# wavey-ai/soundkit

Hardware: AMD Instinct MI355X
Metric: AAC-LC 1024-sample frames/s (whole node) + xrealtime, batch=4096 48 kHz stereo (higher is better)
Workload: dtype f32 (synthesis f32; s16 between the kernels as in the reference; FIR: the 16-bit samples as 2 x f16 exactly, the f32 taps as 2 x f16 to 2^-24, f32 accumulate; 1.0e-7 rel. RMS vs f64)

## Files before the change

soundkit_amd/csrc/fir_bf16.hip:

```cpp
#include "sk_device.h"

#include <cstdlib>
#include <type_traits>

namespace sk {

namespace {

typedef float f32x4 __attribute__((ext_vector_type(4)));
typedef __bf16 bf16x8 __attribute__((ext_vector_type(8)));
typedef uint32_t u32x4 __attribute__((ext_vector_type(4)));
typedef uint32_t u32x2 __attribute__((ext_vector_type(2)));

constexpr int kRing = 192;
constexpr int kPlaneBytes = 2 * kRing;
__host__ __device__ constexpr int row_bytes(int planes) { return planes * kPlaneBytes + 32; }
constexpr int kWindows = 10;
__device__ constexpr int kProducts[kWindows] = {1, 3, 6, 6, 6, 6, 6, 3, 3, 1};
__host__ __device__ constexpr int products_of(int s, bool in16) { return in16 && kProducts[s] > 5 ? 5 : kProducts[s]; }
__device__ constexpr int kProductsF16[kWindows] = {kFirProductsF16[0], kFirProductsF16[1], kFirProductsF16[2], kFirProductsF16[3], kFirProductsF16[4],
                                                     kFirProductsF16[5], kFirProductsF16[6], kFirProductsF16[7], kFirProductsF16[8], kFirProductsF16[9]};
__host__ __device__ constexpr int products_of(int s, bool in16, bool f16) { return f16 ? kProductsF16[s] : products_of(s, in16); }
#ifndef SK_BF_AHEAD
#define SK_BF_AHEAD 3
#endif
constexpr int kAhead = SK_BF_AHEAD;

__host__ __device__ constexpr int ring_index(int rho) { return ((rho % kRing) + kRing) % kRing; }

template <bool PACKED>
__device__ __forceinline__ size_t row_base_offset(const FirArgs &a, uint32_t row) {
    if (!PACKED) return (size_t)row * a.in_stride;
    const uint32_t sh = a.in_ch - 1;
    return (size_t)(row >> sh) * a.in_group_stride + (size_t)((row & sh) << 10);
}

template <bool PACKED>
__device__ __forceinline__ size_t time_offset(const FirArgs &a, uint32_t i) {
    return PACKED ? (size_t)(i >> 10) * a.in_block_stride + (size_t)(i & 1023) : (size_t)i;
}

__device__ __forceinline__ void split_pair(float x0, float x1, uint32_t &p1, uint32_t &p2, uint32_t &p3) {
    const uint32_t u0 = __float_as_uint(x0), u1 = __float_as_uint(x1);
    p1 = __builtin_amdgcn_perm(u1, u0, 0x07060302u);
    const float r0 = x0 - __uint_as_float(u0 & 0xffff0000u), r1 = x1 - __uint_as_float(u1 & 0xffff0000u);
    const uint32_t v0 = __float_as_uint(r0), v1 = __float_as_uint(r1);
    p2 = __builtin_amdgcn_perm(v1, v0, 0x07060302u);
    const float s0 = r0 - __uint_as_float(v0 & 0xffff0000u), s1 = r1 - __uint_as_float(v1 & 0xffff0000u);
    p3 = __builtin_amdgcn_perm(__float_as_uint(s1), __float_as_uint(s0), 0x07060302u);
}

__device__ __forceinline__ void split_pair16(uint32_t u, uint32_t &p1, uint32_t &p2) {
    const uint32_t m = u & 0xff00ff00u;
    const float a0 = (float)(int)(int16_t)(m & 0xffffu), a1 = (float)((int)m >> 16);
    const float b0 = (float)(u & 0xffu), b1 = (float)((u >> 16) & 0xffu);
    p1 = __builtin_amdgcn_perm(__float_as_uint(a1), __float_as_uint(a0), 0x07060302u);
    p2 = __builtin_amdgcn_perm(__float_as_uint(b1), __float_as_uint(b0), 0x07060302u);
}

__device__ __forceinline__ void split_pair16_f16(uint32_t u, uint32_t &p1, uint32_t &p2) { dev_split_pair16_f16(u, p1, p2); }

template <bool IN16>
struct Stage {
    using Elem = std::conditional_t<IN16, int16_t, float>;
    using Vec = std::conditional_t<IN16, u32x2, f32x4>;
    const Elem *base[4];
    uint32_t ok_mask;
    Vec v[2 * kAhead];
};

template <bool ALIGNED, bool PACKED, bool IN16>
__device__ __forceinline__ void stage_init(const FirArgs &a, int lane, uint32_t row0, Stage<IN16> &st) {
    st.ok_mask = 0;
    if (ALIGNED) {
#pragma unroll
        for (int ld = 0; ld < 4; ++ld) {
            const uint32_t r = row0 + 4 * ld + (lane >> 4);
            const bool ok = r < a.rows;
            const uint32_t phys = a.row_map ? a.row_map[ok ? r : 0] : (ok ? r : 0);
            if constexpr (IN16) st.base[ld] = a.in16 + row_base_offset<PACKED>(a, phys) + 4 * (lane & 15);
            else st.base[ld] = a.in + row_base_offset<PACKED>(a, phys) + 4 * (lane & 15);
            if (ok) st.ok_mask |= 1u << ld;
        }
    }
}

template <bool ALIGNED, bool PACKED, bool INTERIOR = false, bool IN16 = false>
__device__ __forceinline__ void stage_issue(const FirArgs &a, int lane, uint32_t row0, int64_t n, Stage<IN16> &st, int half, int slot) {
    using Vec = typename Stage<IN16>::Vec;
    using Elem = typename Stage<IN16>::Elem;
    if (ALIGNED) {
        const int64_t c0 = n - a.in_origin;
        const bool inside = c0 >= 0 && c0 + 64 <= (int64_t)a.in_frames;
        const bool one_block = !PACKED || (((uint32_t)c0 & 1023u) + 64u <= 1024u);
        if (INTERIOR || __builtin_expect(inside && one_block, 1)) {
            const size_t off = time_offset<PACKED>(a, (uint32_t)c0);
#pragma unroll
            for (int e2 = 0; e2 < 2; ++e2) {
                const int ld = 2 * half + e2, sl = 2 * slot + e2;
                st.v[sl] = *reinterpret_cast<const Vec *>(st.base[ld] + off);
            }
        } else {
            asm volatile("; chunk at an edge of the row" ::: "memory");
            const int64_t idx = c0 + 4 * (lane & 15);
            const bool in_range = (uint64_t)idx + 3 < (uint64_t)a.in_frames;
            const ptrdiff_t off = (ptrdiff_t)time_offset<PACKED>(a, (uint32_t)idx) - 4 * (lane & 15);
            const uint32_t sel = in_range ? st.ok_mask : 0u;
#pragma unroll
            for (int e2 = 0; e2 < 2; ++e2) {
                const int ld = 2 * half + e2, sl = 2 * slot + e2;
                const Elem *src = ((sel >> ld) & 1u) ? st.base[ld] + off : reinterpret_cast<const Elem *>(a.zeros) + 4 * lane;
                st.v[sl] = *reinterpret_cast<const Vec *>(src);
            }
        }
    } else if constexpr (!IN16) {
        const int64_t idx = n + lane - a.in_origin;
        const bool in_range = idx >= 0 && idx < (int64_t)a.in_frames;
        const size_t off = time_offset<PACKED>(a, (uint32_t)idx);
#pragma unroll
        for (int e2 = 0; e2 < 2; ++e2) {
            const int ld = 2 * half + e2, sl = 2 * slot + e2;
#pragma unroll
            for (int e = 0; e < 4; ++e) {
                const uint32_t r = row0 + 4 * ld + e;
                const bool ok = in_range && r < a.rows;
                const uint32_t phys = a.row_map ? a.row_map[r < a.rows ? r : 0] : r;
                st.v[sl][e] = ok ? a.in[row_base_offset<PACKED>(a, phys) + off] : 0.0f;
            }
        }
    }
}

template <bool ALIGNED, bool IN16, bool F16 = false>
__device__ __forceinline__ void stage_commit(unsigned char *lds, int lane, int ring_at, const Stage<IN16> &st, int half, int slot) {
#pragma unroll
    for (int e2 = 0; e2 < 2; ++e2) {
        const int ld = 2 * half + e2, sl = 2 * slot + e2;
        if constexpr (IN16) {
            uint32_t p1a, p2a, p1b, p2b;
            if constexpr (F16) {
                split_pair16_f16(st.v[sl][0], p1a, p2a);
                split_pair16_f16(st.v[sl][1], p1b, p2b);
            } else {
                split_pair16(st.v[sl][0], p1a, p2a);
                split_pair16(st.v[sl][1], p1b, p2b);
            }
            unsigned char *dst = lds + (4 * ld + (lane >> 4)) * row_bytes(2) + 2 * (ring_at + 4 * (lane & 15));
            *reinterpret_cast<u32x2 *>(dst) = (u32x2){p1a, p1b};
            *reinterpret_cast<u32x2 *>(dst + kPlaneBytes) = (u32x2){p2a, p2b};
        } else if (ALIGNED) {
            uint32_t p1a, p2a, p3a, p1b, p2b, p3b;
            split_pair(st.v[sl][0], st.v[sl][1], p1a, p2a, p3a);
            split_pair(st.v[sl][2], st.v[sl][3], p1b, p2b, p3b);
            unsigned char *dst = lds + (4 * ld + (lane >> 4)) * row_bytes(3) + 2 * (ring_at + 4 * (lane & 15));
            *reinterpret_cast<u32x2 *>(dst) = (u32x2){p1a, p1b};
            *reinterpret_cast<u32x2 *>(dst + kPlaneBytes) = (u32x2){p2a, p2b};
            *reinterpret_cast<u32x2 *>(dst + 2 * kPlaneBytes) = (u32x2){p3a, p3b};
        } else {
#pragma unroll
            for (int e = 0; e < 4; ++e) {
                uint32_t p1, p2, p3;
                split_pair(st.v[sl][e], 0.0f, p1, p2, p3);
                unsigned char *dst = lds + (4 * ld + e) * row_bytes(3) + 2 * (ring_at + lane);
                *reinterpret_cast<uint16_t *>(dst) = (uint16_t)p1;
                *reinterpret_cast<uint16_t *>(dst + kPlaneBytes) = (uint16_t)p2;
                *reinterpret_cast<uint16_t *>(dst + 2 * kPlaneBytes) = (uint16_t)p3;
            }
        }
    }
}

struct BFrag {
    u32x4 p[3];
};

__device__ __forceinline__ f32x4 mfma_bf16(const u32x4 &av, const u32x4 &bv, const f32x4 &c) {
    return dev_mfma_bf16(av, bv, c);
}

__device__ __forceinline__ f32x4 mfma_f16(const u32x4 &av, const u32x4 &bv, const f32x4 &c) { return dev_mfma_f16(av, bv, c); }

template <bool ALIGNED, bool PACKED, int OUT16, bool IN16 = false, bool F16 = false>
#ifndef SK_FIR_F16_WAVES
#define SK_FIR_F16_WAVES 3
#endif
__global__ __launch_bounds__(64, F16 ? SK_FIR_F16_WAVES : 2) void k_fir_48k_16k_bf16(FirArgs a, int32_t pair0, int32_t pair_end, int32_t pairs_per_seg,
                                                            uint32_t n_segs, int out_vec) {
    static_assert(!IN16 || ALIGNED, "s16 rows are read four samples at a time");
    static_assert(!F16 || IN16, "the f16 planes exist for s16 rows");
    constexpr int kPlanes = IN16 ? 2 : 3;
    __shared__ __attribute__((aligned(16))) unsigned char lds[16 * row_bytes(kPlanes)];

    const int lane = threadIdx.x;
    const int j = lane & 15, q = lane >> 4;
    const uint32_t group = blockIdx.x / n_segs, seg = blockIdx.x % n_segs;
    const uint32_t row0 = group * 16;
    const int32_t p_begin = pair0 + (int32_t)seg * pairs_per_seg;
    const int32_t p_end = p_begin + pairs_per_seg < pair_end ? p_begin + pairs_per_seg : pair_end;
    if (p_begin >= p_end) return;
    const int32_t p_last = p_end + 3;

    u32x4 af[kWindows][3];
    {
        const u32x4 *src = reinterpret_cast<const u32x4 *>(F16 ? a.afrag_f16 : a.afrag16);
        constexpr int kTapPlanes = F16 ? 2 : 3;
#pragma unroll
        for (int s = 0; s < kWindows; ++s)
#pragma unroll
            for (int k = 0; k < kTapPlanes; ++k) af[s][k] = src[(s * kTapPlanes + k) * 64 + lane];
    }

    Stage<IN16> st;
    stage_init<ALIGNED, PACKED, IN16>(a, lane, row0, st);

    const int64_t n_begin = (int64_t)96 * p_begin;
#pragma unroll
    for (int c = -2; c < 0; ++c) {
        stage_issue<ALIGNED, PACKED, false, IN16>(a, lane, row0, n_begin + 64 * c, st, 0, 0);
        stage_issue<ALIGNED, PACKED, false, IN16>(a, lane, row0, n_begin + 64 * c, st, 1, 1);
        stage_commit<ALIGNED, IN16, F16>(lds, lane, ring_index(64 * c), st, 0, 0);
        stage_commit<ALIGNED, IN16, F16>(lds, lane, ring_index(64 * c), st, 1, 1);
    }
#pragma unroll
    for (int i = 0; i < kAhead; ++i) stage_issue<ALIGNED, PACKED, false, IN16>(a, lane, row0, n_begin + 64 * (i >> 1), st, i & 1, i % kAhead);

    const uint32_t out_row = row0 + j;
    float *out_ptr = OUT16 ? nullptr
                           : a.out + (size_t)(out_row < a.rows ? out_row : 0) * a.out_stride +
                                 ((a.out_off && out_row < a.rows) ? a.out_off[out_row] : 0);

    const unsigned char *b_base = lds + j * row_bytes(kPlanes) + 16 * q;
    const unsigned char *b_base_wrap = b_base - (q >= 2 ? 2 * kRing : 0);
    auto read_b = [&](int rho) __attribute__((always_inline)) {
        BFrag f;
        const unsigned char *src = (ring_index(rho) + 32 > kRing ? b_base_wrap : b_base) + 2 * ring_index(rho);
#pragma unroll
        for (int p = 0; p < kPlanes; ++p) f.p[p] = *reinterpret_cast<const u32x4 *>(src + p * kPlaneBytes);
        return f;
    };

    const bool row_exists = out_row < a.rows;
    constexpr bool to_s16 = OUT16 != 0;
    float *out_lane = to_s16 ? nullptr : out_ptr + 4 * q;
    int16_t *out16_ptr = to_s16 ? a.out16 + (size_t)((row_exists ? out_row : 0) / (OUT16 ? OUT16 : 1)) * a.out16_stride * OUT16 : nullptr;
    auto store_tile = [&](auto itag, const f32x4 &vraw, int32_t pair, int parity) __attribute__((always_inline)) {
        const f32x4 v = F16 ? vraw * (1.0f / 2147483648.0f) : (IN16 ? vraw * (1.0f / 32768.0f) : vraw);
        constexpr bool INTERIOR = decltype(itag)::value;
        if (!INTERIOR && (pair < p_begin || pair >= p_end)) return;
        const int32_t rel_tile = 32 * pair + 16 * parity - (int32_t)a.out_first;
        const bool whole = INTERIOR || (out_vec && rel_tile >= 0 && rel_tile + 16 <= (int32_t)a.out_count);
        const bool row_ok = INTERIOR || row_exists;
        const int32_t rel = rel_tile + 4 * q;
        if (!to_s16) {
            if (INTERIOR || __builtin_expect(whole, 1)) {
                if (row_ok) *reinterpret_cast<f32x4 *>(out_lane + rel_tile) = v;
            } else {
                asm volatile("; tile at an edge of the output, or unaligned rows" ::: "memory");
#pragma unroll
                for (int r = 0; r < 4; ++r)
                    if (row_ok && rel + r >= 0 && rel + r < (int32_t)a.out_count) out_ptr[rel + r] = v[r];
            }
            return;
        }
        uint32_t mine01, mine23;
        if constexpr (IN16) {
            mine01 = dev_pack2_s16_scaled<F16 ? 31 : 15>(vraw[0], vraw[1]);
            mine23 = dev_pack2_s16_scaled<F16 ? 31 : 15>(vraw[2], vraw[3]);
        } else {
            mine01 = dev_pack2_s16(v[0], v[1]);
            mine23 = dev_pack2_s16(v[2], v[3]);
        }
        if (OUT16 == 2) {
            const uint32_t other01 = (uint32_t)__builtin_amdgcn_update_dpp(0, (int)mine01, 0xB1, 0xF, 0xF, true);
            const uint32_t other23 = (uint32_t)__builtin_amdgcn_update_dpp(0, (int)mine23, 0xB1, 0xF, 0xF, true);
            uint32_t w[4];
            w[0] = (mine01 & 0xffffu) | (other01 << 16);
            w[1] = (mine01 >> 16) | (other01 & 0xffff0000u);
            w[2] = (mine23 & 0xffffu) | (other23 << 16);
            w[3] = (mine23 >> 16) | (other23 & 0xffff0000u);
            if ((j & 1) == 0 && row_ok) {
                uint32_t *dst = reinterpret_cast<uint32_t *>(out16_ptr) + rel;
                if (INTERIOR || __builtin_expect(whole, 1)) {
                    *reinterpret_cast<u32x4 *>(dst) = (u32x4){w[0], w[1], w[2], w[3]};
                } else {
                    asm volatile("; tile at an edge of the output, or unaligned rows" ::: "memory");
#pragma unroll
                    for (int r = 0; r < 4; ++r)
                        if (rel + r >= 0 && rel + r < (int32_t)a.out_count) dst[r] = w[r];
                }
            }
        } else if (row_ok) {
            int16_t *dst = out16_ptr + rel;
            if (INTERIOR || __builtin_expect(whole, 1)) {
                *reinterpret_cast<u32x2 *>(dst) = (u32x2){mine01, mine23};
            } else {
                asm volatile("; tile at an edge of the output, or unaligned rows" ::: "memory");
#pragma unroll
                for (int r = 0; r < 4; ++r)
                    if (rel + r >= 0 && rel + r < (int32_t)a.out_count) dst[r] = (int16_t)((r < 2 ? mine01 : mine23) >> (16 * (r & 1)));
            }
        }
    };

    f32x4 acc[2][4];
#pragma unroll
    for (int par = 0; par < 2; ++par)
#pragma unroll
        for (int b = 0; b < 4; ++b) acc[par][b] = (f32x4){0.f, 0.f, 0.f, 0.f};

    BFrag bcur = read_b(-128);

    auto period = [&](auto ktag, auto itag, int32_t P, int64_t n_body) __attribute__((always_inline)) {
        constexpr int K = decltype(ktag)::value;
        constexpr bool INTERIOR = decltype(itag)::value;
#pragma unroll
        for (int wi = 0; wi < 3; ++wi) {
            const int step = 3 * K + wi;
            {
                __builtin_amdgcn_sched_barrier(0);
                stage_commit<ALIGNED, IN16, F16>(lds, lane, ring_index(64 * (step >> 1)), st, step & 1, step % kAhead);
                stage_issue<ALIGNED, PACKED, INTERIOR, IN16>(a, lane, row0, n_body + 64 * ((step + kAhead) >> 1), st,
                                                             (step + kAhead) & 1, step % kAhead);
            }
#pragma unroll
            for (int par = 0; par < 2; ++par) {
                const int t = 32 * step;
                const int rho_next = par == 0 ? t - 80 : t + 32 - 128;
                const BFrag bnext = read_b(rho_next);
#pragma unroll
                for (int prod = 0; prod < 6; ++prod) {
                    constexpr int hk[6] = {0, 1, 0, 1, 2, 0};
                    constexpr int xk[6] = {0, 0, 1, 1, 0, 2};
#pragma unroll
                    for (int d = 0; d < 4; ++d) {
                        const int s = 3 * d + wi;
                        if (s >= kWindows || prod >= products_of(s, IN16, F16)) continue;
                        f32x4 &c = acc[par][(K - d + 4) & 3];
                        const f32x4 c0 = (s == 0 && prod == 0) ? (f32x4){0.f, 0.f, 0.f, 0.f} : c;
                        if constexpr (F16) c = mfma_f16(af[s][hk[prod]], bcur.p[xk[prod]], c0);
                        else c = mfma_bf16(af[s][hk[prod]], bcur.p[xk[prod]], c0);
                    }
                }
                if (wi == 1 && par == 0) {
                    store_tile(itag, acc[0][(K + 1) & 3], P - 3, 0);
                    store_tile(itag, acc[1][(K + 1) & 3], P - 3, 1);
                }
                bcur = bnext;
            }
            if (INTERIOR) {
                int mfmas = 0;
#pragma unroll
                for (int d = 0; d < 4; ++d)
                    if (3 * d + wi < kWindows) mfmas += 2 * products_of(3 * d + wi, IN16, F16);
#pragma unroll
                for (int g = 0; g < mfmas; ++g) {
                    __builtin_amdgcn_sched_group_barrier(0x008, 1, 0);
                    __builtin_amdgcn_sched_group_barrier(0x002, 2, 0);
                }
            }
        }
    };

    using K0 = std::integral_constant<int, 0>;
    using K1 = std::integral_constant<int, 1>;
    using K2 = std::integral_constant<int, 2>;
    using K3 = std::integral_constant<int, 3>;
    const bool chunks_in_blocks = !PACKED || ((uint32_t)(n_begin - a.in_origin) & 63u) == 0;
    auto is_interior = [&](int32_t P0) {
        const int64_t n_body = (int64_t)96 * P0;
        const int64_t c_first = n_body + 64 * (kAhead >> 1) - a.in_origin, c_end = n_body + 64 * ((11 + kAhead) >> 1) + 64 - a.in_origin;
        const int64_t rel_first = (int64_t)32 * (P0 - 3) - (int64_t)a.out_first, rel_end = (int64_t)32 * P0 + 32 - (int64_t)a.out_first;
        return ALIGNED && chunks_in_blocks && c_first >= 0 && c_end <= (int64_t)a.in_frames && P0 - 3 >= p_begin && P0 < p_end &&
               out_vec && rel_first >= 0 && rel_end <= (int64_t)a.out_count && row0 + 16 <= a.rows;
    };
    auto general_body = [&](int32_t P0) __attribute__((always_inline)) {
        const int64_t n_body = (int64_t)96 * P0;
        if (P0 + 0 < p_last) period(K0{}, std::false_type{}, P0 + 0, n_body);
        if (P0 + 1 < p_last) period(K1{}, std::false_type{}, P0 + 1, n_body);
        if (P0 + 2 < p_last) period(K2{}, std::false_type{}, P0 + 2, n_body);
        if (P0 + 3 < p_last) period(K3{}, std::false_type{}, P0 + 3, n_body);
    };
    int32_t P0 = p_begin;
    for (; P0 < p_last && !is_interior(P0); P0 += 4) general_body(P0);
    for (; P0 < p_last && is_interior(P0); P0 += 4) {
        const int64_t n_body = (int64_t)96 * P0;
        period(K0{}, std::true_type{}, P0 + 0, n_body);
        period(K1{}, std::true_type{}, P0 + 1, n_body);
        period(K2{}, std::true_type{}, P0 + 2, n_body);
        period(K3{}, std::true_type{}, P0 + 3, n_body);
    }
    for (; P0 < p_last; P0 += 4) general_body(P0);
}

}

static bool fir_bf16_supported(const FirArgs &a) {
    const int64_t end_pair = ((int64_t)a.out_first + a.out_count + 31) / 32;
    return a.afrag16 != nullptr && end_pair <= 0x7ffffff0ll / 96 && a.out_count <= 0x7fffff00u;
}

hipError_t launch_fir_48k_16k(const FirArgs &a, hipStream_t s) {
    if (a.rows == 0 || a.out_count == 0) return hipSuccess;
    if (!fir_bf16_supported(a)) return hipErrorInvalidValue;
    const uint32_t groups = (a.rows + 15) / 16;
    const int64_t first_pair = ((int64_t)a.out_first / 32) & ~(int64_t)3;
    const int64_t end_pair = ((int64_t)a.out_first + a.out_count + 31) / 32;
    if (end_pair > 0x7ffffff0ll / 96 || a.out_count > 0x7fffff00u) return hipErrorInvalidValue;
    const uint32_t pairs = (uint32_t)(end_pair - first_pair);
    static const bool f16_rows = [] { const char *v = std::getenv("SK_FIR_S16_BF16"); return !(v && v[0] == '1'); }();
    const uint32_t waves_target = (a.in16 && a.afrag_f16 && f16_rows) ? 1024u * SK_FIR_F16_WAVES : 2048u;
    uint32_t n_segs = (waves_target + groups - 1) / groups;
    const uint32_t max_segs = pairs / 16 ? pairs / 16 : 1;
    if (n_segs > max_segs) n_segs = max_segs;
    uint32_t pps = (pairs + n_segs - 1) / n_segs;
    pps = (pps + 3) & ~3u;
    n_segs = (pairs + pps - 1) / pps;

    const bool strides_ok = a.in_block ? (a.in_block % 4 == 0 && a.in_block_stride % 4 == 0 && a.in_group_stride % 4 == 0)
                                       : (a.in_stride % 4 == 0);
    const bool aligned = ((a.in_origin & 3) == 0) && strides_ok && (a.in_frames % 4 == 0) &&
                         (a.in16 ? (((uintptr_t)a.in16 & 7) == 0) : (((uintptr_t)a.in & 15) == 0));
    if (a.out16 && (a.out16_ch < 1 || a.out16_ch > 2 || a.out_off || a.rows % a.out16_ch)) return hipErrorInvalidValue;
    const int out_vec = a.out16 ? ((a.out_first % 4 == 0) && (a.out16_stride * a.out16_ch) % 8 == 0 && (((uintptr_t)a.out16 & 15) == 0))
                                : ((a.out_first % 4 == 0) && (a.out_stride % 4 == 0) && (((uintptr_t)a.out & 15) == 0) &&
                                   a.out_off == nullptr);
    const bool packed = a.in_block != 0;
    if (packed && (a.in_block != 1024 || a.in_ch < 1 || a.in_ch > 2)) return hipErrorInvalidValue;
    const dim3 grid(groups * n_segs), block(64);
#define SK_FIR_LAUNCH(AL, PK, O16)                                                                                 \
    hipLaunchKernelGGL((k_fir_48k_16k_bf16<AL, PK, O16>), grid, block, 0, s, a, (int32_t)first_pair, (int32_t)end_pair, \
                       (int32_t)pps, n_segs, out_vec)
    if (a.in16) {
        if (!packed || !aligned) return hipErrorInvalidValue;
        const bool use_f16 = f16_rows;
#define SK_FIR_LAUNCH16(O16, F)                                                                                                    \
    hipLaunchKernelGGL((k_fir_48k_16k_bf16<true, true, O16, true, F>), grid, block, 0, s, a, (int32_t)first_pair, (int32_t)end_pair, \
                       (int32_t)pps, n_segs, out_vec)
        if (use_f16 && a.afrag_f16) {
            if (!a.out16) SK_FIR_LAUNCH16(0, true);
            else if (a.out16_ch == 2) SK_FIR_LAUNCH16(2, true);
            else SK_FIR_LAUNCH16(1, true);
        } else {
            if (!a.out16) SK_FIR_LAUNCH16(0, false);
            else if (a.out16_ch == 2) SK_FIR_LAUNCH16(2, false);
            else SK_FIR_LAUNCH16(1, false);
        }
#undef SK_FIR_LAUNCH16
    } else if (a.out16) {
        if (!packed) return hipErrorInvalidValue;
        if (aligned && a.out16_ch == 2) SK_FIR_LAUNCH(true, true, 2);
        else if (aligned) SK_FIR_LAUNCH(true, true, 1);
        else if (a.out16_ch == 2) SK_FIR_LAUNCH(false, true, 2);
        else SK_FIR_LAUNCH(false, true, 1);
    } else if (aligned && packed) SK_FIR_LAUNCH(true, true, 0);
    else if (aligned) SK_FIR_LAUNCH(true, false, 0);
    else if (packed) SK_FIR_LAUNCH(false, true, 0);
    else SK_FIR_LAUNCH(false, false, 0);
#undef SK_FIR_LAUNCH
    return hipGetLastError();
}

}
```

soundkit_amd/csrc/sk_device.h:

```cpp
#pragma once
#include <hip/hip_runtime.h>
#include <stdint.h>

#include "../../include/soundkit_amd.h"
#include "mp3_codebook_blob.h"

namespace sk {

struct SynthEntry {
    uint32_t off1024;
    uint32_t win;
};

struct SynthTask {
    uint32_t state;
    uint32_t begin;
    uint32_t count;
    uint32_t pad;
};

struct SynthTables {
    const float2 *tw_long;
    const float2 *tw_short;
    const float2 *w64;
    const float2 *w512;
    const float *win;
};

struct SynthArgs {
    const float *coeffs;
    float *pcm;
    int16_t *pcm16;
    float *delay;
    uint8_t *prev_shape;
    const SynthTask *tasks;
    const SynthEntry *entries;
    uint32_t n_tasks;
    uint32_t only_long;
    SynthTables t;
};

struct FrameSpan {
    uint32_t off1024;
    uint32_t channels;
};

hipError_t launch_aac_synth(const SynthArgs &a, hipStream_t s);
struct TailArgs {
    SynthArgs s;
    const uint32_t *afrag_f16;
    int16_t *out16;
    size_t out_stride;
    size_t stream_stride;
};
hipError_t launch_aac_tail(const TailArgs &ta, hipStream_t s);
hipError_t launch_aac_synth_pairs(const SynthArgs &a, bool with_short, hipStream_t s);
hipError_t launch_reset_streams(float *delay, uint8_t *shape, uint32_t *pns, const uint32_t *ids, uint32_t n, hipStream_t s);
hipError_t launch_zero_spans(float *base, const uint32_t *ids, uint32_t n, uint32_t span_floats, hipStream_t s);
hipError_t launch_frames_to_s16(const float *planar, int16_t *out, const FrameSpan *frames, uint32_t n, hipStream_t s);
hipError_t launch_dequantize(const int16_t *q, const int16_t *sf, float *out, size_t n, const float *pow43,
                             const float *sftab, hipStream_t s);

hipError_t launch_pcm_convert(int op, const void *in, void *out, size_t n, hipStream_t s);
hipError_t launch_interleave(const void *planar, void *out, size_t frames, uint32_t ch, int elem_bytes, hipStream_t s);
hipError_t launch_deinterleave(const void *in, void *planar, size_t frames, uint32_t ch, int elem_bytes, hipStream_t s);
hipError_t launch_deinterleave_s24(const uint8_t *in, int32_t *planar, size_t frames, uint32_t ch, hipStream_t s);
hipError_t launch_bytes_to_f32_planar(int variant, int fmt, const uint8_t *in, size_t frames, uint32_t ch, float *planar,
                                      hipStream_t s);
hipError_t launch_f32_planar_to_bytes(int fmt, const float *planar, size_t frames, uint32_t ch, uint8_t *out,
                                      hipStream_t s);
hipError_t launch_downmix_mono(const float *planar, size_t frames, uint32_t ch, float *mono, hipStream_t s);
hipError_t launch_exact_to_i16(int fmt, const uint8_t *in, size_t samples, uint8_t *out, hipStream_t s);
hipError_t launch_f32_planar_to_bytes_batch(int fmt, const float *planar, size_t batch, size_t plane_stride, size_t frames,
                                            uint32_t ch, uint8_t *out, hipStream_t s);

#ifdef __HIPCC__
__device__ __forceinline__ int dev_float_sample_to_i16(float x) {
    const float f = isfinite(x) ? fminf(fmaxf(x, -1.0f), 1.0f) : 0.0f;
    const double scaled = f < 0.0f ? (double)f * 32768.0 : (double)f * 32767.0;
    const int r = (int)round(scaled);
    return r < -32768 ? -32768 : (r > 32767 ? 32767 : r);
}

__device__ __forceinline__ int dev_float_sample_to_i16_f32(float x) {
    const float m = isfinite(x) ? fminf(fabsf(x), 1.0f) : 0.0f;
    const float a = m * 32768.0f;
    const float k = floorf(a);
    const float d = a - k;
    const int ki = (int)k;
    const int neg = ki + (d >= 0.5f ? 1 : 0);
    const int pos = ki + ((d - 0.5f >= m) ? 1 : 0) - ((d + 0.5f < m) ? 1 : 0);
    return x < 0.0f ? -neg : pos;
}
__device__ __forceinline__ int dev_float_sample_to_i16_v2(float x) {
    const float m = isfinite(x) ? fminf(fabsf(x), 1.0f) : 0.0f;
    const float a = m * 32768.0f;
    const float d = __builtin_amdgcn_fractf(a);
    const int ki = (int)a;
    const float mm = x < 0.0f ? 0.0f : m;
    const int r = ki + ((d - 0.5f >= mm) ? 1 : 0) - ((d + 0.5f < mm) ? 1 : 0);
    return x < 0.0f ? -r : r;
}
__device__ __forceinline__ int dev_float_sample_to_i16_presat(float x) {
    const float y = __builtin_fmaf(x, 0.0f, x);
    const double X = (double)y;
    const double half = __builtin_copysign(0.5, X);
    const double h = __builtin_fma(__builtin_fabs(X), -0.5, half);
    const double t = __builtin_fma(X, 32767.5, h);
    int k;
    asm("v_cvt_i32_f64 %0, %1" : "=v"(k) : "v"(t));
    return k;
}
__device__ __forceinline__ int dev_guarded_sample_to_i16_presat(float y) {
    const double X = (double)y;
    const double half = __builtin_copysign(0.5, X);
    const double h = __builtin_fma(__builtin_fabs(X), -0.5, half);
    const double t = __builtin_fma(X, 32767.5, h);
    int k;
    asm("v_cvt_i32_f64 %0, %1" : "=v"(k) : "v"(t));
    return k;
}
__device__ __forceinline__ uint32_t dev_pack2_s16(float lo, float hi) {
    typedef short s16x2_t __attribute__((ext_vector_type(2)));
    typedef float f32x2_t __attribute__((ext_vector_type(2)));
    const f32x2_t x = {lo, hi};
    const f32x2_t y = __builtin_elementwise_fma(x, (f32x2_t){0.0f, 0.0f}, x);
    const s16x2_t p = __builtin_amdgcn_cvt_pk_i16(dev_guarded_sample_to_i16_presat(y.x), dev_guarded_sample_to_i16_presat(y.y));
    return __builtin_bit_cast(uint32_t, p);
}

template <int EXP>
__device__ __forceinline__ int dev_scaled_sample_to_i16_presat(float acc) {
    constexpr double kScale = 1.0 / (double)(1ull << EXP);
    const double X = (double)acc;
    const double half = __builtin_copysign(0.5, X);
    const double h = __builtin_fma(__builtin_fabs(X), -0.5 * kScale, half);
    const double t = __builtin_fma(X, 32767.5 * kScale, h);
    int k;
    asm("v_cvt_i32_f64 %0, %1" : "=v"(k) : "v"(t));
    return k;
}
template <int EXP>
__device__ __forceinline__ uint32_t dev_pack2_s16_scaled(float lo, float hi) {
    typedef short s16x2_t __attribute__((ext_vector_type(2)));
    const s16x2_t p = __builtin_amdgcn_cvt_pk_i16(dev_scaled_sample_to_i16_presat<EXP>(lo), dev_scaled_sample_to_i16_presat<EXP>(hi));
    return __builtin_bit_cast(uint32_t, p);
}

typedef uint32_t sk_u32x4 __attribute__((ext_vector_type(4)));
typedef float sk_f32x4 __attribute__((ext_vector_type(4)));
__device__ __forceinline__ void dev_split_pair16_f16(uint32_t u, uint32_t &p1, uint32_t &p2) {
    typedef float f32x2 __attribute__((ext_vector_type(2)));
    const f32x2 f = {(float)(short)(u & 0xffffu), (float)((int)u >> 16)};
    const auto a = __builtin_amdgcn_cvt_pkrtz(f.x, f.y);
    const f32x2 r = f - (f32x2){(float)a[0], (float)a[1]};
    p1 = __builtin_bit_cast(uint32_t, a);
    p2 = __builtin_bit_cast(uint32_t, __builtin_amdgcn_cvt_pkrtz(r.x, r.y));
}
__device__ __forceinline__ sk_f32x4 dev_mfma_f16(const sk_u32x4 &av, const sk_u32x4 &bv, const sk_f32x4 &c) {
#if SK_MFMA_K16
    typedef _Float16 f16x4 __attribute__((ext_vector_type(4)));
    typedef uint32_t u32x2 __attribute__((ext_vector_type(2)));
    const sk_f32x4 t = __builtin_amdgcn_mfma_f32_16x16x16f16(__builtin_bit_cast(f16x4, (u32x2){av.x, av.y}), __builtin_bit_cast(f16x4, (u32x2){bv.x, bv.y}), c, 0, 0, 0);
    return __builtin_amdgcn_mfma_f32_16x16x16f16(__builtin_bit_cast(f16x4, (u32x2){av.z, av.w}), __builtin_bit_cast(f16x4, (u32x2){bv.z, bv.w}), t, 0, 0, 0);
#else
    typedef _Float16 f16x8 __attribute__((ext_vector_type(8)));
    return __builtin_amdgcn_mfma_f32_16x16x32_f16(__builtin_bit_cast(f16x8, av), __builtin_bit_cast(f16x8, bv), c, 0, 0, 0);
#endif
}
__device__ __forceinline__ sk_f32x4 dev_mfma_bf16(const sk_u32x4 &av, const sk_u32x4 &bv, const sk_f32x4 &c) {
#if SK_MFMA_K16
    typedef short s16x4 __attribute__((ext_vector_type(4)));
    typedef uint32_t u32x2 __attribute__((ext_vector_type(2)));
    const sk_f32x4 t = __builtin_amdgcn_mfma_f32_16x16x16bf16_1k(__builtin_bit_cast(s16x4, (u32x2){av.x, av.y}), __builtin_bit_cast(s16x4, (u32x2){bv.x, bv.y}), c, 0, 0, 0);
    return __builtin_amdgcn_mfma_f32_16x16x16bf16_1k(__builtin_bit_cast(s16x4, (u32x2){av.z, av.w}), __builtin_bit_cast(s16x4, (u32x2){bv.z, bv.w}), t, 0, 0, 0);
#else
    typedef __bf16 bf16x8 __attribute__((ext_vector_type(8)));
    return __builtin_amdgcn_mfma_f32_16x16x32_bf16(__builtin_bit_cast(bf16x8, av), __builtin_bit_cast(bf16x8, bv), c, 0, 0, 0);
#endif
}
__device__ constexpr int kFirProductsF16[10] = {1, 3, 3, 3, 3, 3, 3, 3, 1, 1};
#endif

struct FirArgs {
    const float *in;
    const int16_t *in16;
    float *out;
    int16_t *out16;
    size_t out16_stride;
    uint32_t out16_ch;
    const float *zeros;
    const uint32_t *afrag16;
    const uint32_t *afrag_f16;
    const float *taps;
    size_t in_stride, out_stride;
    uint32_t in_block, in_ch;
    size_t in_block_stride, in_group_stride;
    const uint32_t *row_map;
    const uint32_t *out_off;
    uint32_t rows;
    uint32_t in_frames;
    int32_t in_origin;
    uint32_t out_first;
    uint32_t out_count;
};
hipError_t launch_fir_48k_16k(const FirArgs &a, hipStream_t s);

struct SincArgs {
    const float *in;
    float *out;
    const float *sincs;
    const double *set_starts;
    const uint32_t *set_count;
    const uint32_t *row_set;
    uint32_t starts_stride;
    double step;
    const uint32_t *row_map;
    const uint32_t *out_off;
    size_t in_stride, out_stride;
    uint32_t rows, in_frames, out_count;
    int32_t in_origin;
    uint32_t n_sets;
    void *scratch;
    size_t scratch_bytes;
    int exact;
};
hipError_t launch_sinc_resample(const SincArgs &a, hipStream_t s);
uint32_t sinc_rows_per_block();
size_t sinc_mfma_scratch_bytes(uint32_t n_sets, uint32_t out_count, double step);

struct SincS16Args {
    const int16_t *in16;
    size_t stream_stride, frame_stride;
    uint32_t channels;
    uint32_t rows;
    uint32_t in_frames;
    int16_t *out16;
    float *out32;
    size_t out_stride;
    const float *sincs;
    const double *set_starts;
    const uint32_t *set_count;
    uint32_t starts_stride;
    double step;
    uint32_t out_count;
    void *scratch;
    size_t scratch_bytes;
};
hipError_t launch_sinc_rows_s16(const SincS16Args &a, hipStream_t s);

struct RowCopy {
    uint64_t src_off, dst_off;
    uint32_t count;
    uint32_t via_s16;
    uint32_t pieces = 1;
    uint32_t src_stride = 0;
};
hipError_t launch_row_copies(const float *src_base, float *dst_base, const RowCopy *jobs, uint32_t n_jobs, hipStream_t s);

constexpr uint32_t kMp3StateFloats = 1664;
struct Mp3Args {
    const float *xr;
    float *pcm;
    int16_t *pcm16;
    uint32_t planar_stride;
    float *state;
    const SynthTask *tasks;
    const SynthEntry *entries;
    uint32_t n_tasks;
    const float *imdct;
    const float *matrix;
    const float *window;
    const float *cs_ca;
};
hipError_t launch_mp3_hybrid(const Mp3Args &a, hipStream_t s);

struct Mp12Entry {
    uint32_t record;
    uint32_t pcm_off;
};
struct Mp12Args {
    const sk_mpa_frame_record *records;
    const uint32_t *bytes;
    float *pcm;
    int16_t *pcm16;
    uint32_t planar_stride;
    float *state;
    const SynthTask *tasks;
    const Mp12Entry *entries;
    uint32_t n_tasks;
    const float *matrix;
    const float *window;
    const float *scf;
};
hipError_t launch_mp12_synth(const Mp12Args &a, hipStream_t s);

constexpr uint32_t kMp3Rates = 9;
constexpr uint32_t kMp3BandRow = 40;
constexpr uint32_t kMp3Pow43 = 8208;
struct Mp3RequantRecord {
    uint32_t off;
    uint8_t slot, channels, flags, reserved;
    sk_mp3_requant_channel ch[2];
};
static_assert(sizeof(Mp3RequantRecord) % 4 == 0 && sizeof(Mp3RequantRecord) <= 256, "one word per lane");
struct Mp3RequantArgs {
    const Mp3RequantRecord *records;
    const int16_t *is;
    float *xr;
    uint32_t n;
    const float *pow43;
    const float *root4;
    const float *is_k;
    const uint16_t *bands;
    const uint8_t *pretab;
    const uint32_t *line_map;
};
hipError_t launch_mp3_requant(const Mp3RequantArgs &a, hipStream_t s);

static_assert(kMp3BlobRates == kMp3Rates, "one region table per band-table slot");
struct Mp3EntropyItem {
    uint32_t frame;
    uint32_t row;
    uint32_t record;
    uint8_t gr, ch, reserved[2];
};
struct Mp3EntropyCell {
    uint8_t scalefac_l[22];
    uint8_t scalefac_s[13][3];
    uint8_t preflag, intensity_scale, reserved;
    uint16_t part2_bits, nonzero_lines, part3_bits, reserved2;
    int32_t status;
};
static_assert(sizeof(Mp3EntropyCell) == 76, "packed by hand");
struct Mp3EntropyArgs {
    const uint32_t *blob;
    uint32_t lds_words;
    const sk_mp3_frame_item *frames;
    const uint8_t *bytes;
    const Mp3EntropyItem *items;
    uint32_t n_items;
    uint32_t lane_shift;
    int16_t *is;
    Mp3RequantRecord *records;
    Mp3EntropyCell *cells;
    int32_t *status;
};
hipError_t launch_mp3_entropy(const Mp3EntropyArgs &a, hipStream_t s);

}
#include "aac_entropy_core.h"
namespace sk {
constexpr int EC_SKIPPED = -199;
struct EntropyUnit {
    uint32_t word_offset;
    uint32_t byte_len;
    uint32_t off1024;
    uint32_t entry[2];
    uint32_t task;
};
struct EntropyTask {
    uint32_t stream, first, count;
    int32_t sf_index;
    uint32_t channels;
};
struct EntropyArgs {
    sk_ec::Tables t;
    const uint8_t *lds_blob;
    uint32_t lds_bytes;
    uint32_t lds_meta_off, lds_lut_off, lds_tuple_off, lds_sf_off, lds_swb_off, lds_pow_off;
    const uint32_t *words;
    const EntropyUnit *units;
    const EntropyTask *tasks;
    uint32_t n_tasks;
    uint32_t *pns_state;
    float *coeffs;
    SynthEntry *entries;
    int32_t *status;
    uint32_t n_units;
    sk_ec::Scratch *side;
    uint32_t *pns_start;
    uint32_t lane_shift;
    const uint32_t *order;
    const sk_ec::WireUnit *wire;
    const int16_t *quant;
};
hipError_t launch_aac_entropy_parallel(const EntropyArgs &a, hipStream_t s);

enum PackMode : uint8_t {
    kPackPlain = 0,
    kPackViaS16 = 1,
    kPackDirect = 2,
    kPackFromQ = 3,
    kPackPlainF32 = 4,
};
struct PackJob {
    const float *src0, *src1;
    uint8_t *dst;
    uint32_t frames;
    uint8_t ch_in, ch_out, bits, mode;
};
hipError_t launch_pack_jobs(const PackJob *jobs, uint32_t n_jobs, uint32_t max_frames, hipStream_t s);

constexpr uint32_t kPcmSliceSamples = 4096;
constexpr uint32_t kPcmCutFrames = 16;
struct PcmDirectJob {
    const uint8_t *src;
    uint8_t *dst;
    uint32_t frames;
    uint8_t fmt_in;
    uint8_t fmt_out;
    uint8_t ch_in, ch_out;
    uint32_t exact;
    uint32_t pad;
};
hipError_t launch_pcm_direct(const PcmDirectJob *jobs, uint32_t n_jobs, uint32_t max_samples , hipStream_t s);
struct PcmIngestJob {
    const uint8_t *src;
    float *dst0, *dst1;
    uint32_t frames;
    uint8_t fmt, ch, pad[2];
};
hipError_t launch_pcm_ingest(const PcmIngestJob *jobs, uint32_t n_jobs, uint32_t max_samples, hipStream_t s);

constexpr uint32_t kWideSliceFrames = 512;
constexpr uint8_t kWidePlanar = 0xff;
constexpr uint32_t kWideNoPeak = 0xffffffffu;
struct WideJob {
    const void *src;
    void *dst;
    uint64_t src_stride;
    uint64_t dst_stride;
    uint32_t frames;
    uint32_t peak;
    uint8_t fmt_in;
    uint8_t fmt_out;
    uint8_t ch_in, ch_out;
    uint32_t pad;
};
hipError_t launch_pcm_wide(const WideJob *jobs, uint32_t n_jobs, uint32_t n_peak_jobs, uint32_t max_frames, bool bytes_in, uint32_t *peaks,
                           hipStream_t s);
hipError_t launch_pcm_wide_one(const WideJob &job, uint32_t *peaks, hipStream_t s);
struct PcmWideIngestJob {
    const uint8_t *src;
    float *dst;
    uint64_t row_stride;
    uint32_t frames;
    uint8_t fmt, ch, pad[2];
};
hipError_t launch_pcm_wide_ingest(const PcmWideIngestJob *jobs, uint32_t n_jobs, uint32_t max_frames, hipStream_t s);

struct AiffElemJob {
    const uint8_t *src;
    uint8_t *dst;
    uint32_t samples;
    uint32_t enc;
};
hipError_t launch_aiff_elem(const AiffElemJob *jobs, uint32_t n_jobs, uint32_t max_samples, hipStream_t s);
struct AiffImaUnit {
    const uint8_t *src;
    uint8_t *dst;
    uint32_t groups;
    uint32_t pad;
};
struct AiffImaStream {
    uint32_t first_unit, n_units;
    int16_t predictor[2];
    uint8_t step_index[2];
    uint8_t channels;
    uint8_t pad;
};
hipError_t launch_aiff_ima4(const AiffImaStream *streams, uint32_t n_streams, const AiffImaUnit *units, uint32_t *states_out, hipStream_t s);

struct FlacFrame {
    uint32_t byte_offset;
    uint32_t byte_len;
    uint32_t block_size;
    uint32_t ws_offset;
    uint64_t out_offset;
    uint32_t sub0;
    uint8_t header_bytes, channels, assignment, bits;
};
struct FlacSubframe {
    int16_t coef[32];
    uint8_t kind;
    uint8_t order, shift, wasted;
    uint32_t ws_offset, block_size, frame;
};
enum : uint8_t { kFlacConstant = 0, kFlacVerbatim = 1, kFlacPredict = 2 };
enum : uint32_t { kFlacOutContract = 0, kFlacOutI32 = 1, kFlacOutI16Clamp = 2 };
hipError_t launch_flac_residual(const FlacFrame *frames, const uint32_t *by_length, uint32_t n_frames, const uint8_t *bytes, uint32_t bytes_len,
                                int32_t *ws, FlacSubframe *subs, int32_t *status, hipStream_t s);
hipError_t launch_flac_restore(const FlacSubframe *subs, uint32_t n_subs, int32_t *ws, const int32_t *status, hipStream_t s);
hipError_t launch_flac_output(const FlacFrame *frames, uint32_t n_frames, const FlacSubframe *subs, const int32_t *ws, const int32_t *status,
                              uint8_t *out, uint32_t mode, hipStream_t s);

}
```

Baseline: 267.1 million.

## Use scalar base plus 32-bit lane offsets for FIR row loads, trim s16 split and store

Adds a non-WIDE addressing mode in which each FIR block holds a single scalar row-group base pointer plus 32-bit per-lane byte offsets, instead of four 64-bit per-lane pointers. This is meant to cut VGPR usage and 64-bit address arithmetic in the load path. The host picks this mode when spans fit in 32 bits and there is no row_map or out_off, and an environment variable can force the old path. The change also rewrites the s16 to f16 residual split with fma_mix instructions and uses a single DPP exchange for the interior stereo s16 store. These add inline-asm constraints and a dependence on the host-side span check being correct.

```diff
diff --git a/soundkit_amd/csrc/fir_bf16.hip b/soundkit_amd/csrc/fir_bf16.hip
--- a/soundkit_amd/csrc/fir_bf16.hip
+++ b/soundkit_amd/csrc/fir_bf16.hip
@@ -60,45 +60,63 @@
 
 __device__ __forceinline__ void split_pair16_f16(uint32_t u, uint32_t &p1, uint32_t &p2) { dev_split_pair16_f16(u, p1, p2); }
 
-template <bool IN16>
+template <bool IN16, bool WIDE>
 struct Stage {
     using Elem = std::conditional_t<IN16, int16_t, float>;
     using Vec = std::conditional_t<IN16, u32x2, f32x4>;
-    const Elem *base[4];
+    std::conditional_t<WIDE, const Elem *, uint32_t> base[4];
+    const Elem *gbase;
     uint32_t ok_mask;
     Vec v[2 * kAhead];
 };
 
-template <bool ALIGNED, bool PACKED, bool IN16>
-__device__ __forceinline__ void stage_init(const FirArgs &a, int lane, uint32_t row0, Stage<IN16> &st) {
+template <bool ALIGNED, bool PACKED, bool IN16, bool WIDE>
+__device__ __forceinline__ void stage_init(const FirArgs &a, int lane, uint32_t row0, Stage<IN16, WIDE> &st) {
+    using Elem = typename Stage<IN16, WIDE>::Elem;
     st.ok_mask = 0;
+    st.gbase = nullptr;
     if (ALIGNED) {
+        const Elem *in;
+        if constexpr (IN16) in = a.in16;
+        else in = a.in;
+        if constexpr (!WIDE) st.gbase = in + row_base_offset<PACKED>(a, row0);
 #pragma unroll
         for (int ld = 0; ld < 4; ++ld) {
             const uint32_t r = row0 + 4 * ld + (lane >> 4);
             const bool ok = r < a.rows;
-            const uint32_t phys = a.row_map ? a.row_map[ok ? r : 0] : (ok ? r : 0);
-            if constexpr (IN16) st.base[ld] = a.in16 + row_base_offset<PACKED>(a, phys) + 4 * (lane & 15);
-            else st.base[ld] = a.in + row_base_offset<PACKED>(a, phys) + 4 * (lane & 15);
+            if constexpr (WIDE) {
+                const uint32_t phys = a.row_map ? a.row_map[ok ? r : 0] : (ok ? r : 0);
+                st.base[ld] = in + row_base_offset<PACKED>(a, phys) + 4 * (lane & 15);
+            } else {
+                const size_t rel = row_base_offset<PACKED>(a, ok ? r : row0) - row_base_offset<PACKED>(a, row0);
+                st.base[ld] = (uint32_t)((rel + 4 * (lane & 15)) * sizeof(Elem));
+            }
             if (ok) st.ok_mask |= 1u << ld;
         }
     }
 }
 
-template <bool ALIGNED, bool PACKED, bool INTERIOR = false, bool IN16 = false>
-__device__ __forceinline__ void stage_issue(const FirArgs &a, int lane, uint32_t row0, int64_t n, Stage<IN16> &st, int half, int slot) {
-    using Vec = typename Stage<IN16>::Vec;
-    using Elem = typename Stage<IN16>::Elem;
+template <bool ALIGNED, bool PACKED, bool INTERIOR = false, bool IN16 = false, bool WIDE = true>
+__device__ __forceinline__ void stage_issue(const FirArgs &a, int lane, uint32_t row0, int64_t n, Stage<IN16, WIDE> &st, int half, int slot) {
+    using Vec = typename Stage<IN16, WIDE>::Vec;
+    using Elem = typename Stage<IN16, WIDE>::Elem;
     if (ALIGNED) {
         const int64_t c0 = n - a.in_origin;
         const bool inside = c0 >= 0 && c0 + 64 <= (int64_t)a.in_frames;
         const bool one_block = !PACKED || (((uint32_t)c0 & 1023u) + 64u <= 1024u);
         if (INTERIOR || __builtin_expect(inside && one_block, 1)) {
             const size_t off = time_offset<PACKED>(a, (uint32_t)c0);
+            auto chunk = (const __attribute__((address_space(1))) unsigned char *)(st.gbase + off);
+            if constexpr (!WIDE) asm("" : "+s"(chunk));
 #pragma unroll
             for (int e2 = 0; e2 < 2; ++e2) {
                 const int ld = 2 * half + e2, sl = 2 * slot + e2;
-                st.v[sl] = *reinterpret_cast<const Vec *>(st.base[ld] + off);
+                if constexpr (WIDE) st.v[sl] = *reinterpret_cast<const Vec *>(st.base[ld] + off);
+                else {
+                    uint32_t lane_off = st.base[ld];
+                    asm("" : "+v"(lane_off));
+                    st.v[sl] = *(const __attribute__((address_space(1))) Vec *)(chunk + lane_off);
+                }
             }
         } else {
             asm volatile("; chunk at an edge of the row" ::: "memory");
@@ -109,7 +127,10 @@
 #pragma unroll
             for (int e2 = 0; e2 < 2; ++e2) {
                 const int ld = 2 * half + e2, sl = 2 * slot + e2;
-                const Elem *src = ((sel >> ld) & 1u) ? st.base[ld] + off : reinterpret_cast<const Elem *>(a.zeros) + 4 * lane;
+                const Elem *row;
+                if constexpr (WIDE) row = st.base[ld];
+                else row = reinterpret_cast<const Elem *>(reinterpret_cast<const unsigned char *>(st.gbase) + st.base[ld]);
+                const Elem *src = ((sel >> ld) & 1u) ? row + off : reinterpret_cast<const Elem *>(a.zeros) + 4 * lane;
                 st.v[sl] = *reinterpret_cast<const Vec *>(src);
             }
         }
@@ -131,8 +152,8 @@
     }
 }
 
-template <bool ALIGNED, bool IN16, bool F16 = false>
-__device__ __forceinline__ void stage_commit(unsigned char *lds, int lane, int ring_at, const Stage<IN16> &st, int half, int slot) {
+template <bool ALIGNED, bool IN16, bool F16 = false, bool WIDE = true>
+__device__ __forceinline__ void stage_commit(unsigned char *lds, int lane, int ring_at, const Stage<IN16, WIDE> &st, int half, int slot) {
 #pragma unroll
     for (int e2 = 0; e2 < 2; ++e2) {
         const int ld = 2 * half + e2, sl = 2 * slot + e2;
@@ -180,7 +201,7 @@
 
 __device__ __forceinline__ f32x4 mfma_f16(const u32x4 &av, const u32x4 &bv, const f32x4 &c) { return dev_mfma_f16(av, bv, c); }
 
-template <bool ALIGNED, bool PACKED, int OUT16, bool IN16 = false, bool F16 = false>
+template <bool ALIGNED, bool PACKED, int OUT16, bool IN16 = false, bool F16 = false, bool WIDE = true>
 #ifndef SK_FIR_F16_WAVES
 #define SK_FIR_F16_WAVES 3
 #endif
@@ -188,6 +209,7 @@
                                                             uint32_t n_segs, int out_vec) {
     static_assert(!IN16 || ALIGNED, "s16 rows are read four samples at a time");
     static_assert(!F16 || IN16, "the f16 planes exist for s16 rows");
+    static_assert(WIDE || ALIGNED, "lane offsets exist for rows read four samples at a time");
     constexpr int kPlanes = IN16 ? 2 : 3;
     __shared__ __attribute__((aligned(16))) unsigned char lds[16 * row_bytes(kPlanes)];
 
@@ -210,7 +232,7 @@
             for (int k = 0; k < kTapPlanes; ++k) af[s][k] = src[(s * kTapPlanes + k) * 64 + lane];
     }
 
-    Stage<IN16> st;
+    Stage<IN16, WIDE> st;
     stage_init<ALIGNED, PACKED, IN16>(a, lane, row0, st);
 
     const int64_t n_begin = (int64_t)96 * p_begin;
@@ -270,7 +292,14 @@
             mine01 = dev_pack2_s16(v[0], v[1]);
             mine23 = dev_pack2_s16(v[2], v[3]);
         }
-        if (OUT16 == 2) {
+        if constexpr (OUT16 == 2 && INTERIOR) {
+            const bool odd = (j & 1) != 0;
+            const uint32_t keep = odd ? mine23 : mine01, send = odd ? mine01 : mine23;
+            const uint32_t got = (uint32_t)__builtin_amdgcn_update_dpp(0, (int)send, 0xB1, 0xF, 0xF, true);
+            const uint32_t left = odd ? got : keep, right = odd ? keep : got;
+            uint32_t *dst = reinterpret_cast<uint32_t *>(out16_ptr) + rel + (odd ? 2 : 0);
+            *reinterpret_cast<u32x2 *>(dst) = (u32x2){(left & 0xffffu) | (right << 16), (left >> 16) | (right & 0xffff0000u)};
+        } else if (OUT16 == 2) {
             const uint32_t other01 = (uint32_t)__builtin_amdgcn_update_dpp(0, (int)mine01, 0xB1, 0xF, 0xF, true);
             const uint32_t other23 = (uint32_t)__builtin_amdgcn_update_dpp(0, (int)mine23, 0xB1, 0xF, 0xF, true);
             uint32_t w[4];
@@ -427,15 +456,40 @@
     const bool packed = a.in_block != 0;
     if (packed && (a.in_block != 1024 || a.in_ch < 1 || a.in_ch > 2)) return hipErrorInvalidValue;
     const dim3 grid(groups * n_segs), block(64);
-#define SK_FIR_LAUNCH(AL, PK, O16)                                                                                 \
-    hipLaunchKernelGGL((k_fir_48k_16k_bf16<AL, PK, O16>), grid, block, 0, s, a, (int32_t)first_pair, (int32_t)end_pair, \
+    static const bool force_wide = [] { const char *v = std::getenv("SK_FIR_WIDE"); return v && v[0] == '1'; }();
+    const bool wide = [&] {
+        if (force_wide || a.row_map || a.out_off) return true;
+        constexpr uint64_t kLimit = 0xffffff00ull, kStride = 1ull << 32;
+        const uint64_t in_elem = a.in16 ? sizeof(int16_t) : sizeof(float);
+        uint64_t in_span;
+        if (packed) {
+            if (a.in_group_stride >= kStride || a.in_block_stride >= kStride) return true;
+            in_span = 15 * (uint64_t)a.in_group_stride + 1024 + (uint64_t)(a.in_frames >> 10) * a.in_block_stride + 1024;
+        } else {
+            if (a.in_stride >= kStride) return true;
+            in_span = 15 * (uint64_t)a.in_stride + a.in_frames;
+        }
+        if ((in_span + 128) * in_elem > kLimit) return true;
+        const uint64_t out_pitch = a.out16 ? (uint64_t)a.out16_stride * a.out16_ch * sizeof(int16_t) : (uint64_t)a.out_stride * sizeof(float);
+        if ((a.out16 ? a.out16_stride : a.out_stride) >= kStride) return true;
+        return 15 * out_pitch + ((uint64_t)a.out_count + 64) * 4 > kLimit;
+    }();
+#define SK_FIR_LAUNCH_W(AL, PK, O16, I16, F, W)                                                                                      \
+    hipLaunchKernelGGL((k_fir_48k_16k_bf16<AL, PK, O16, I16, F, W>), grid, block, 0, s, a, (int32_t)first_pair, (int32_t)end_pair, \
                        (int32_t)pps, n_segs, out_vec)
+#define SK_FIR_LAUNCH(AL, PK, O16)                                          \
+    do {                                                                    \
+        if (AL && !wide) SK_FIR_LAUNCH_W(AL, PK, O16, false, false, !AL);   \
+        else SK_FIR_LAUNCH_W(AL, PK, O16, false, false, true);              \
+    } while (0)
     if (a.in16) {
         if (!packed || !aligned) return hipErrorInvalidValue;
         const bool use_f16 = f16_rows;
-#define SK_FIR_LAUNCH16(O16, F)                                                                                                    \
-    hipLaunchKernelGGL((k_fir_48k_16k_bf16<true, true, O16, true, F>), grid, block, 0, s, a, (int32_t)first_pair, (int32_t)end_pair, \
-                       (int32_t)pps, n_segs, out_vec)
+#define SK_FIR_LAUNCH16(O16, F)                                        \
+    do {                                                               \
+        if (!wide) SK_FIR_LAUNCH_W(true, true, O16, true, F, false);   \
+        else SK_FIR_LAUNCH_W(true, true, O16, true, F, true);          \
+    } while (0)
         if (use_f16 && a.afrag_f16) {
             if (!a.out16) SK_FIR_LAUNCH16(0, true);
             else if (a.out16_ch == 2) SK_FIR_LAUNCH16(2, true);
@@ -457,6 +511,7 @@
     else if (packed) SK_FIR_LAUNCH(false, true, 0);
     else SK_FIR_LAUNCH(false, false, 0);
 #undef SK_FIR_LAUNCH
+#undef SK_FIR_LAUNCH_W
     return hipGetLastError();
 }
 
diff --git a/soundkit_amd/csrc/sk_device.h b/soundkit_amd/csrc/sk_device.h
--- a/soundkit_amd/csrc/sk_device.h
+++ b/soundkit_amd/csrc/sk_device.h
@@ -150,12 +150,12 @@
 typedef uint32_t sk_u32x4 __attribute__((ext_vector_type(4)));
 typedef float sk_f32x4 __attribute__((ext_vector_type(4)));
 __device__ __forceinline__ void dev_split_pair16_f16(uint32_t u, uint32_t &p1, uint32_t &p2) {
-    typedef float f32x2 __attribute__((ext_vector_type(2)));
-    const f32x2 f = {(float)(short)(u & 0xffffu), (float)((int)u >> 16)};
-    const auto a = __builtin_amdgcn_cvt_pkrtz(f.x, f.y);
-    const f32x2 r = f - (f32x2){(float)a[0], (float)a[1]};
-    p1 = __builtin_bit_cast(uint32_t, a);
-    p2 = __builtin_bit_cast(uint32_t, __builtin_amdgcn_cvt_pkrtz(r.x, r.y));
+    const float f0 = (float)(short)(u & 0xffffu), f1 = (float)((int)u >> 16);
+    p1 = __builtin_bit_cast(uint32_t, __builtin_amdgcn_cvt_pkrtz(f0, f1));
+    uint32_t r;
+    asm("v_fma_mixlo_f16 %0, -%1, 1.0, %2 op_sel:[0,0,0] op_sel_hi:[1,0,0]" : "=v"(r) : "v"(p1), "v"(f0));
+    asm("v_fma_mixhi_f16 %0, -%1, 1.0, %2 op_sel:[1,0,0] op_sel_hi:[1,0,0]" : "+v"(r) : "v"(p1), "v"(f1));
+    p2 = r;
 }
 __device__ __forceinline__ sk_f32x4 dev_mfma_f16(const sk_u32x4 &av, const sk_u32x4 &bv, const sk_f32x4 &c) {
 #if SK_MFMA_K16
```

Result: no change. 268.8 million (median of 6 runs) (+0.6%).
